# yusuke1127/RoboManipBaselines

Measured on AMD Instinct MI355X. Metric: env-steps/s (whole node) + policy-inference us/step, MujocoUR5eCable x N ACT, higher is better.
Workload: dtype f64 physics + fp32 policy

## Files before the change

### include/rmbx.h

```cpp
#ifndef RMBX_H_
#define RMBX_H_

#include <stddef.h>
#include <stdint.h>

#ifdef __cplusplus
extern "C" {
#endif

#define RMBX_OK 0
#define RMBX_ERR_ARG -1
#define RMBX_ERR_HIP -2
#define RMBX_ERR_STATE -3

#define RMBX_ABI_VERSION 2

int rmbx_abi_version(void);
const char* rmbx_last_error(void);
int rmbx_device_count(int* count);

int rmbx_act_ensemble(const float* new_chunk, const uint8_t* push, const uint8_t* active,
                      float* hist, int32_t* hist_len, int32_t* hist_head,
                      const double* w_table, const double* dn_scale, const double* dn_sub,
                      const double* dn_add, double* out, int n_env, int chunk, int adim,
// ... 368 lines not shown
int rmbx_split_bf16x3(const float* x, void* planes, long long n, void* stream);
int rmbx_split_f16x2(const float* w, int N, int K, void* planes, float* scale, void* stream);
int rmbx_linear_f16x3(const float* a, long long lda, const void* w_planes, long long ldw, long long w_plane_stride,
                      const float* w_scale, const float* bias, float* c, long long ldc, int M, int N, int K, int relu,
                      void* stream);
int rmbx_linear_f16x3_batched(const float* a, long long lda, long long a_bs, const void* w_planes, long long ldw,
                              long long w_plane_stride, long long w_bs, const float* w_scale, long long ws_bs,
                              const float* bias, float* c, long long ldc, long long c_bs, int batch, int M, int N,
                              int K, int relu, void* stream);
int rmbx_linear_f16x3_presplit(const void* a_planes, long long lda, long long a_plane_stride, const float* a_rinv,
                               const void* w_planes, long long ldw, long long w_plane_stride, const float* w_scale,
                               const float* bias, const float* res, float* c, long long ldc, int M, int N, int K,
                               int relu, void* stream);
int rmbx_linear_f16x3_presplit_split(const void* a_planes, long long lda, long long a_plane_stride, const float* a_rinv,
                                     const float* a_norm, const void* w_planes, long long ldw, long long w_plane_stride,
                                     const float* w_scale, float w_norm_max, float b_abs_max, const float* bias,
                                     int relu, void* out_planes, long long ldo, long long out_plane_stride,
                                     float* out_rinv, int M, int N, int K, void* stream);
int rmbx_linear_f16x3_presplit_batched(const void* a_planes, long long lda, long long a_plane_stride, long long a_bs,
                                       const float* a_rinv, long long r_bs, const void* w_planes, long long ldw,
                                       long long w_plane_stride, long long w_bs, const float* w_scale, long long ws_bs,
                                       const float* bias, float* c, long long ldc, long long c_bs, int batch, int M,
                                       int N, int K, int relu, void* stream);
int rmbx_conv3x3_f16x3_patch(const float* in, int N, int H, int W, int C, const void* w_planes,
                             long long w_plane_stride, const float* w_scale, const float* bias, const float* res,
                             float* out, int Cout, int relu, void* stream);
int rmbx_conv2d_f16x3(const float* in, int N, int H, int W, int C, const void* w_planes, const float* w_scale,
                      const float* bias, const float* res, float* out, int Cout, int KH, int KW, int stride, int pad,
                      int relu, void* stream);
int rmbx_attention_f32x6(const float* q, const float* k, const float* v, float* out, int B, int heads, int Lq, int Lk,
                         long long q_bstride, int q_rstride, long long k_bstride, int k_rstride, long long v_bstride,
                         int v_rstride, float scale, void* stream);
int rmbx_attention_f16x3(const float* q, const float* k, const float* v, float* out, int* redo, int B, int heads,
                         int Lq, int Lk, long long q_bstride, int q_rstride, long long k_bstride, int k_rstride,
                         long long v_bstride, int v_rstride, float scale, void* stream);
int rmbx_groupnorm_act(const float* x, const float* weight, const float* bias, float* out, int B, int C, int T,
                       int groups, float eps, int mish, void* stream);
int rmbx_add_layernorm(const void* x, const void* r, const float* weight, const float* bias, void* out,
                       int rows, int D, float eps, int dtype, void* stream);
int rmbx_add_layernorm_pos(const void* x, const void* r, const float* weight, const float* bias, void* out,
                           const void* pos, int pos_rows, void* out_pos, int rows, int D, float eps, int dtype,
                           void* stream);
int rmbx_add_layernorm_split(const float* x, const float* r, const float* weight, const float* bias, float* out,
                             void* y_planes, float* y_rinv, float* y_norm, const float* pos, int pos_rows,
                             float* out_pos, void* pos_planes, float* pos_rinv, int rows, int D, float eps,
                             void* stream);
// ... 68 lines not shown
```

### robomanipbaselines_amd/_native.py

```python

import ctypes
import os

import numpy as np

_LIB_PATH = os.path.join(os.path.dirname(os.path.abspath(__file__)), "_lib",
                         f"librmbx_{os.environ['RMBX_LIB_VARIANT']}.so" if os.environ.get("RMBX_LIB_VARIANT")
                         else "librmbx.so")

_c_int = ctypes.c_int
_c_p = ctypes.c_void_p
_c_sz = ctypes.c_size_t
_c_d = ctypes.c_double

SIGNATURES = {
    "rmbx_abi_version": (_c_int, []),
    "rmbx_last_error": (ctypes.c_char_p, []),
    "rmbx_device_count": (_c_int, [_c_p]),
    "rmbx_act_ensemble": (
        _c_int,
        [_c_p] * 11 + [_c_int, _c_int, _c_int, _c_int, _c_p],
    ),
    "rmbx_cable_reward": (_c_int, [_c_p] * 5 + [_c_int, _c_int, _c_p]),
    "rmbx_door_reward": (_c_int, [_c_p, _c_p, _c_p, _c_p, _c_int, _c_d, _c_d, _c_p]),
# ... 59 lines not shown
    "rmbx_conv2d_direct_f32": (_c_int, [_c_p] + [_c_int] * 4 + [_c_p] * 3 + [_c_int] * 5 + [_c_p]),
    "rmbx_split_bf16x3": (_c_int, [_c_p, _c_p, ctypes.c_longlong, _c_p]),
    "rmbx_split_f16x2": (_c_int, [_c_p, _c_int, _c_int, _c_p, _c_p, _c_p]),
    "rmbx_linear_f16x3": (_c_int, [_c_p, ctypes.c_longlong, _c_p, ctypes.c_longlong, ctypes.c_longlong, _c_p, _c_p,
                                   _c_p, ctypes.c_longlong, _c_int, _c_int, _c_int, _c_int, _c_p]),
    "rmbx_linear_f16x3_batched": (_c_int, [_c_p, ctypes.c_longlong, ctypes.c_longlong, _c_p, ctypes.c_longlong,
                                           ctypes.c_longlong, ctypes.c_longlong, _c_p, ctypes.c_longlong, _c_p, _c_p,
                                           ctypes.c_longlong, ctypes.c_longlong] + [_c_int] * 5 + [_c_p]),
    "rmbx_conv3x3_f16x3_patch": (_c_int, [_c_p] + [_c_int] * 4 + [_c_p, ctypes.c_longlong] + [_c_p] * 4
                                 + [_c_int, _c_int, _c_p]),
    "rmbx_conv2d_f16x3": (_c_int, [_c_p] + [_c_int] * 4 + [_c_p] * 5 + [_c_int] * 6 + [_c_p]),
    "rmbx_add_layernorm": (_c_int, [_c_p] * 5 + [_c_int, _c_int, ctypes.c_float, _c_int, _c_p]),
    "rmbx_groupnorm_act": (_c_int, [_c_p] * 4 + [_c_int] * 4 + [ctypes.c_float, _c_int, _c_p]),
    "rmbx_add_layernorm_split": (_c_int, [_c_p] * 9 + [_c_int, _c_p, _c_p, _c_p, _c_int, _c_int, ctypes.c_float, _c_p]),
    "rmbx_linear_f16x3_presplit_split": (_c_int, [_c_p, ctypes.c_longlong, ctypes.c_longlong, _c_p, _c_p, _c_p,
                                                  ctypes.c_longlong, ctypes.c_longlong, _c_p, ctypes.c_float,
                                                  ctypes.c_float, _c_p, _c_int, _c_p, ctypes.c_longlong,
                                                  ctypes.c_longlong, _c_p, _c_int, _c_int, _c_int, _c_p]),
    "rmbx_linear_f16x3_presplit_batched": (_c_int, [_c_p, ctypes.c_longlong, ctypes.c_longlong, ctypes.c_longlong, _c_p,
                                                    ctypes.c_longlong, _c_p, ctypes.c_longlong, ctypes.c_longlong,
                                                    ctypes.c_longlong, _c_p, ctypes.c_longlong, _c_p, _c_p,
                                                    ctypes.c_longlong, ctypes.c_longlong, _c_int, _c_int, _c_int, _c_int,
                                                    _c_int, _c_p]),
    "rmbx_wino4_input_split": (_c_int, [_c_p, _c_int, _c_int, _c_int, _c_int, _c_p, _c_p, _c_p]),
    "rmbx_linear_f16x3_presplit": (_c_int, [_c_p, ctypes.c_longlong, ctypes.c_longlong, _c_p, _c_p, ctypes.c_longlong,
                                            ctypes.c_longlong, _c_p, _c_p, _c_p, _c_p, ctypes.c_longlong, _c_int, _c_int,
                                            _c_int, _c_int, _c_p]),
    "rmbx_add_layernorm_pos": (_c_int, [_c_p] * 6 + [_c_int, _c_p, _c_int, _c_int, ctypes.c_float, _c_int, _c_p]),
    "rmbx_ddpm_step": (_c_int, [_c_p] * 4 + [_c_sz, _c_p, _c_p]),
    "rmbx_ddim_step": (_c_int, [_c_p] * 3 + [_c_sz, _c_p, _c_int, _c_p]),
    "rmbx_philox_normal": (_c_int, [ctypes.c_uint64, _c_p, _c_p, _c_int, _c_int, _c_p, _c_int, _c_int, _c_int, _c_p]),
    "rmbx_image_perturb": (_c_int, [_c_p, _c_p, _c_p, _c_int, _c_p, ctypes.c_uint64, _c_p, _c_p, _c_int, _c_p, _c_int,
                                    _c_int, _c_int, _c_p]),
    "rmbx_action_perturb": (_c_int, [_c_p] * 7 + [ctypes.c_uint64, _c_p, _c_p, _c_p, _c_int, _c_int, _c_p]),
    "rmbx_resize_crop_u8": (_c_int, [_c_p] + [_c_int] * 10 + [ctypes.c_float, ctypes.c_float, _c_p, _c_int, _c_p]),
    "rmbx_resize_f32": (_c_int, [_c_p, _c_p] + [_c_int] * 5 + [_c_p]),
    "rmbx_pointcloud_fps": (_c_int, [_c_p, _c_p, _c_int, _c_int, _c_int, _c_d, _c_p, _c_p, _c_int, _c_int,
                                     _c_p, _c_p, _c_p, _c_p, _c_p, _c_p, _c_p]),
    "rmbx_sarnn_attention": (_c_int, [_c_p] * 8 + [_c_int] * 4 + [ctypes.c_float, _c_p]),
    "rmbx_sarnn_lstm_step": (_c_int, [_c_p] * 12 + [_c_int] * 4 + [_c_p]),
}


class Camera(ctypes.Structure):

    _fields_ = [("body", ctypes.c_int32), ("width", ctypes.c_int32), ("height", ctypes.c_int32),
# ... 204 lines not shown
```

### robomanipbaselines_amd/csrc/rmbx_gemm.hip

```cpp
#include "rmbx_common.h"

#include <cstdint>
#include <cstdlib>
#include <type_traits>

namespace rmbx {
namespace {

typedef short bf16x8 __attribute__((ext_vector_type(8)));
typedef _Float16 f16x8 __attribute__((ext_vector_type(8)));
typedef float f32x4v __attribute__((ext_vector_type(4)));
typedef __bf16 bf16x2v __attribute__((ext_vector_type(2)));
typedef _Float16 f16x2v __attribute__((ext_vector_type(2)));
typedef float f32x2v __attribute__((ext_vector_type(2)));

constexpr int GM_BM = 256, GM_BN = 128, GM_BK = 32;
constexpr int GM_THREADS = 512;
constexpr int GM_A_PLANE = GM_BM * GM_BK * 2;
constexpr int GM_GROUP = 8;
template <int BN>
constexpr int gm_b_plane() { return BN * GM_BK * 2; }
template <int PC, int BN = 128>
constexpr int gm_stage() { return PC * (GM_A_PLANE + gm_b_plane<BN>()); }
template <int BN>
// ... 1 lines not shown
template <int PC, int BN = 128, int NS = 2>
constexpr int gm_smem() {
  return (NS * gm_stage<PC, BN>() > gm_epi_bytes<BN>() ? NS * gm_stage<PC, BN>() : gm_epi_bytes<BN>()) +
         (PC == 2 ? 1024 + 64 : 0);
}
static_assert(gm_smem<3>() <= 160 * 1024 && gm_smem<2, 128, 3>() <= 160 * 1024 && gm_smem<2, 64, 3>() <= 160 * 1024 &&
                  gm_smem<2, 256, 2>() <= 160 * 1024,
              "the LDS of a CU");

struct GemmArgs {
  const float* A;
  const uint16_t* W;
  const float* bias;
  float* C;
  long long lda, ldc, ldw, wps;
  int M, N, K, relu;
  int tiles_m, tiles_n;
  const float* res;
  int ih, iw, ic, oh, ow, kw, stride, pad;
  int batch;
  long long a_bs, w_bs, c_bs;
  const float* ws;
  long long ws_bs;
};

__device__ __forceinline__ uint32_t pk_bf16(float x, float y) {
  f32x2v v = {x, y};
  return __builtin_bit_cast(uint32_t, __builtin_convertvector(v, bf16x2v));
}

__device__ __forceinline__ void split_pair(float x, float y, uint32_t& p0, uint32_t& p1, uint32_t& p2) {
  p0 = pk_bf16(x, y);
  const float rx = x - __uint_as_float(p0 << 16), ry = y - __uint_as_float(p0 & 0xffff0000u);
  p1 = pk_bf16(rx, ry);
  const float sx = rx - __uint_as_float(p1 << 16), sy = ry - __uint_as_float(p1 & 0xffff0000u);
  p2 = pk_bf16(sx, sy);
}

__device__ __forceinline__ uint32_t pk_f16(float x, float y) {
  f32x2v v = {x, y};
  return __builtin_bit_cast(uint32_t, __builtin_convertvector(v, f16x2v));
}

__device__ __forceinline__ void split_f16_pair(float x, float y, uint32_t& h, uint32_t& l) {
  h = pk_f16(x, y);
  const f16x2v hv = __builtin_bit_cast(f16x2v, h);
  l = pk_f16((x - (float)hv[0]) * 2048.f, (y - (float)hv[1]) * 2048.f);
// ... 33 lines not shown
  R[1] = __builtin_bit_cast(float4, v1);
  R[2] = __builtin_bit_cast(float4, v2);
  R[3] = __builtin_bit_cast(float4, v3);
}

template <bool CONV, int VAR = 0, int PC = 3, int BN = 128>
__global__ void __launch_bounds__(GM_THREADS, 1) gemm_f32x6_kernel(GemmArgs g) {
  static_assert(PC == 3 || PC == 2, "bf16x6 (3 pieces) or f16x3 (2 pieces)");
  static_assert(BN == 128 || ((BN == 64 || BN == 256) && PC == 2), "BN = 64 / 256: the f16x3 form's tiles");
  static_assert(BN != 256 || (VAR & 1024) == 0, "the 256-wide tile runs two stages");
  constexpr int GROUP = ((VAR >> 1) & 3) == 1 ? 4 : ((VAR >> 1) & 3) == 2 ? 16 : GM_GROUP;
  constexpr int STAGE = gm_stage<PC, BN>(), A_BYTES = PC * GM_A_PLANE, B_PLANE = gm_b_plane<BN>();
  constexpr int NJ = BN / 32;
  constexpr int WP = PC * BN / 128;
  constexpr int PPP = BN / 16;
  constexpr int W_OPS = WP, A_OPS = 4, A_ROWS = 2;
  static_assert(A_OPS == 2 * A_ROWS, "two 16-byte loads (8 f32 of one k quarter) per staged row");
  constexpr int NS = (PC == 2 && (VAR & 1024) != 0) ? 3 : 2;
  constexpr int SMEM = gm_smem<PC, BN, NS>();
  __shared__ __attribute__((aligned(16))) unsigned char smem[SMEM];
  const int tid = threadIdx.x, lane = tid & 63, wave = tid >> 6;
  const int wm = wave & 3, wn = wave >> 2;

  const int nblk = gridDim.x, bid = blockIdx.x;
  const int xcd = bid & 7, q = nblk >> 3, r = nblk & 7;
  int lin = (xcd < r ? xcd * (q + 1) : r * (q + 1) + (xcd - r) * q) + (bid >> 3);
  if (g.batch > 1) {
    const int per_item = g.tiles_m * g.tiles_n;
    const int item = lin / per_item;
    lin -= item * per_item;
    g.A += item * g.a_bs;
    g.W += item * g.w_bs;
    g.C += item * g.c_bs;
    if (g.ws) g.ws += item * g.ws_bs;
  }
  const int per_group = GROUP * g.tiles_n;
  const int first_m = (lin / per_group) * GROUP;
  const int gsize = min(g.tiles_m - first_m, GROUP);
  const int in_group = lin - (lin / per_group) * per_group;
  const int tm = first_m + in_group % gsize, tn = in_group / gsize;
  const int m0 = tm * GM_BM, n0 = tn * BN;

  const int aq = tid & 3, arow = tid >> 2;
  const float* ag0 = g.A + (long long)min(m0 + arow, g.M - 1) * g.lda + 8 * aq;
  const float* ag1 = g.A + (long long)min(m0 + arow + 128, g.M - 1) * g.lda + 8 * aq;
  const int aoff0 = arow * 64 + ((aq ^ ((arow >> 2) & 2)) << 4);
  const int aoff1 = (arow + 128) * 64 + ((aq ^ (((arow + 128) >> 2) & 2)) << 4);
  const uint16_t* bsrc[WP];
#pragma unroll
  for (int t = 0; t < WP; ++t) {
    const int i = wave * WP + t, p = i / PPP;
    const int row = (i % PPP) * 16 + (lane >> 2);
    const int sl = (lane & 3) ^ ((row >> 2) & 2);
    bsrc[t] = g.W + p * g.wps + (long long)(n0 + row) * g.ldw + sl * 8;
  }
  auto stage_b = [&](int kt, int buf) {
    if constexpr ((VAR & 512) != 0) {
      if (kt > 0) return;
    }
    unsigned char* base = smem + buf * STAGE + A_BYTES;
#pragma unroll
    for (int t = 0; t < W_OPS; ++t) glds16(bsrc[t] + kt * GM_BK, base + (wave * WP + t) * 1024);
  };
  long long cbase[2] = {0, 0};
  int cy[2] = {0, 0}, cx[2] = {0, 0};
  if constexpr (CONV) {
#pragma unroll
    for (int r2 = 0; r2 < 2; ++r2) {
      const int m = min(m0 + arow + 128 * r2, g.M - 1);
      const int hw = g.oh * g.ow;
      const int img = m / hw, rem = m - img * hw;
      const int oy = rem / g.ow, ox = rem - oy * g.ow;
      cy[r2] = oy * g.stride - g.pad;
      cx[r2] = ox * g.stride - g.pad;
      cbase[r2] = ((long long)(img * g.ih + cy[r2]) * g.iw + cx[r2]) * g.ic + 8 * aq;
    }
  }
// ... 129 lines not shown
          c = __builtin_amdgcn_mfma_f32_16x16x32_bf16(a[i][0], b[nj][0], c, 0, 0, 0);
          acc[2 * h + i][nj] = c;
        }
      }
  };
  auto read_b = [&](bf16x8 (&b)[NJ][PC], int buf) {
    const unsigned char* Bs = smem + buf * STAGE + A_BYTES;
#pragma unroll
    for (int nj = 0; nj < NJ; ++nj) {
      const int off = frag_off(wn * (BN / 2) + nj * 16 + fr);
#pragma unroll
      for (int p = 0; p < PC; ++p) b[nj][p] = *(const bf16x8*)(Bs + p * B_PLANE + off);
    }
  };

  const int KT = g.K / GM_BK;
  constexpr bool SKIPS = (VAR & (256 | 512)) != 0;
  constexpr int LEAD = NS - 1;
  constexpr int SPLIT_WAIT = SKIPS ? 0 : W_OPS + A_OPS;
  constexpr int END_WAIT = SKIPS ? 0 : (NS == 3 ? W_OPS + A_OPS : A_OPS);
  static_assert(SPLIT_WAIT <= 63 && END_WAIT <= 63, "vmcnt holds 6 bits on gfx950");
  static_assert(SKIPS || (END_WAIT < SPLIT_WAIT || NS == 3), "a stage's DMA is retired after the A split");
  auto stage_of = [](int k) { return NS == 2 ? (k & 1) : k % 3; };
  auto k_loop = [&](auto scaled) {
    float4 Ra[4], Rb[4];
    int oka, okb;
    if constexpr (NS == 3) {
      stage_b(0, 0);
      oka = load_a(Ra, 0);
      stage_b(min(1, KT - 1), 1);
      okb = load_a(Rb, min(1, KT - 1));
    } else {
      oka = load_a(Ra, 0);
      stage_b(0, 0);
      okb = load_a(Rb, min(1, KT - 1));
    }
    wait_vm_regs<SPLIT_WAIT>(Ra);
    store_a(Ra, oka, 0, scaled);
    wait_vm<END_WAIT>();
    asm volatile("s_waitcnt lgkmcnt(0)\n\ts_barrier" ::: "memory");
    auto step = [&](int kt, float4 (&Rcur)[4], int& okcur, float4 (&Rnext)[4], int& oknext) {
      const int buf = stage_of(kt), nbuf = stage_of(kt + 1);
      const bool more = kt + 1 < KT;
      stage_b(min(kt + LEAD, KT - 1), stage_of(kt + LEAD));
      oknext = load_a(Rnext, min(kt + 2, KT - 1));
      if constexpr (BN == 256) {
        const unsigned char* S = smem + buf * STAGE;
        f16x8 ah[4], al[4];
#pragma unroll
        for (int mi = 0; mi < 4; ++mi) {
          const int off = frag_off(wm * 64 + mi * 16 + fr);
          ah[mi] = __builtin_bit_cast(f16x8, *(const bf16x8*)(S + off));
          al[mi] = __builtin_bit_cast(f16x8, *(const bf16x8*)(S + GM_A_PLANE + off));
        }
        auto wide_half = [&](int hh) {
#pragma unroll
          for (int q = 0; q < NJ / 2; ++q) {
            const int nj = hh * (NJ / 2) + q;
            const int off = frag_off(wn * (BN / 2) + nj * 16 + fr);
            const f16x8 bh = __builtin_bit_cast(f16x8, *(const bf16x8*)(S + A_BYTES + off));
            const f16x8 bl = __builtin_bit_cast(f16x8, *(const bf16x8*)(S + A_BYTES + B_PLANE + off));
            const f16x8 bsc = bh * (_Float16)0.00048828125f;
#pragma unroll
            for (int mi = 0; mi < 4; ++mi) {
              f32x4v c = acc[mi][nj];
              c = __builtin_amdgcn_mfma_f32_16x16x32_f16(al[mi], bsc, c, 0, 0, 0);
              c = __builtin_amdgcn_mfma_f32_16x16x32_f16(ah[mi], bl, c, 0, 0, 0);
              c = __builtin_amdgcn_mfma_f32_16x16x32_f16(ah[mi], bh, c, 0, 0, 0);
              acc[mi][nj] = c;
            }
          }
        };
        wide_half(0);
        wait_vm_regs<SPLIT_WAIT>(Rcur);
        store_a(Rcur, okcur, nbuf, scaled);
        wide_half(1);
        wait_vm<END_WAIT>();
        if (more) asm volatile("s_waitcnt lgkmcnt(0)\n\ts_barrier" ::: "memory");
// ... 11 lines not shown
        wait_vm_regs<SPLIT_WAIT>(Rcur);
        store_a(Rcur, okcur, nbuf, scaled);
      }
      if constexpr (VAR & 1) __builtin_amdgcn_s_setprio(1);
      half_step(buf, 0, b, bs);
      if constexpr (VAR & 1) __builtin_amdgcn_s_setprio(0);
      if (late) {
        wait_vm_regs<SPLIT_WAIT>(Rcur);
        store_a(Rcur, okcur, nbuf, scaled);
      }
      if constexpr (VAR & 1) __builtin_amdgcn_s_setprio(1);
      half_step(buf, 1, b, bs);
      if constexpr (VAR & 1) __builtin_amdgcn_s_setprio(0);
      wait_vm<END_WAIT>();
      if (more) asm volatile("s_waitcnt lgkmcnt(0)\n\ts_barrier" ::: "memory");
    };
    for (int kt = 0; kt < KT; kt += 2) {
      step(kt, Rb, okb, Ra, oka);
      if (kt + 1 < KT) step(kt + 1, Ra, oka, Rb, okb);
    }
    wait_vm_regs<0>(Ra);
    wait_vm_regs<0>(Rb);
  };
  k_loop(std::false_type{});

  if constexpr (PC == 2) {
    uint32_t b0 = amax0, b1 = amax1;
    b0 = max(b0, (uint32_t)__shfl_xor((int)b0, 1));
    b0 = max(b0, (uint32_t)__shfl_xor((int)b0, 2));
    b1 = max(b1, (uint32_t)__shfl_xor((int)b1, 1));
    b1 = max(b1, (uint32_t)__shfl_xor((int)b1, 2));
    const float m0 = __uint_as_float(b0), m1 = __uint_as_float(b1);
    float inv0 = 1.f, inv1 = 1.f;
    auto row_scale = [](float m, float& sc, float& inv) {
      if ((m > 32768.f || (m > 0.f && m < 0.015625f)) && m <= 3.4e38f) {
        int e;
        frexpf(m, &e);
        sc = ldexpf(1.f, 14 - e);
        inv = ldexpf(1.f, e - 14);
        return true;
      }
      return false;
    };
    const bool need = row_scale(m0, as0, inv0) | row_scale(m1, as1, inv1);
    float* rinv = reinterpret_cast<float*>(smem + SMEM - 1024 - 64);
    int* flag = reinterpret_cast<int*>(smem + SMEM - 64);
    if (aq == 0) {
      rinv[arow] = inv0;
      rinv[arow + 128] = inv1;
    }
    const unsigned long long bal = __ballot(need);
    if (lane == 0) flag[wave] = bal != 0ull;
    asm volatile("s_waitcnt vmcnt(0) lgkmcnt(0)\n\ts_barrier" ::: "memory");
    int any = 0;
#pragma unroll
    for (int w = 0; w < 8; ++w) any |= flag[w];
    if (any) {
      zero_acc();
      k_loop(std::true_type{});
    }
    if (any) {
#pragma unroll
      for (int i = 0; i < 4; ++i)
#pragma unroll
        for (int e = 0; e < 4; ++e) {
          const float inv = rinv[wm * 64 + i * 16 + 4 * fs + e];
#pragma unroll
          for (int j = 0; j < NJ; ++j) acc[i][j][e] *= inv;
        }
    }
  }

  if constexpr ((VAR & 16) != 0) {
    asm volatile("s_waitcnt lgkmcnt(0)\n\ts_barrier" ::: "memory");
    constexpr int WC = BN / 2 < 64 ? BN / 2 : 64, PITCH = WC + 4;
    constexpr int LPR = WC / 4, RPI = 64 / LPR;
    constexpr int NPASS = (BN / 2) / WC, NJP = NJ / NPASS;
    float* T = reinterpret_cast<float*>(smem) + wave * (64 * PITCH);
#pragma unroll
    for (int pass = 0; pass < NPASS; ++pass) {
    if (pass > 0) asm volatile("s_waitcnt lgkmcnt(0)" ::: "memory");
#pragma unroll
    for (int mi = 0; mi < 4; ++mi)
#pragma unroll
      for (int q = 0; q < NJP; ++q)
#pragma unroll
        for (int e = 0; e < 4; ++e) T[(mi * 16 + 4 * fs + e) * PITCH + q * 16 + fr] = acc[mi][pass * NJP + q][e];
    asm volatile("s_waitcnt lgkmcnt(0)" ::: "memory");
    const int c4 = (lane % LPR) * 4;
    const int n = n0 + wn * (BN / 2) + pass * WC + c4;
    float4 bn = make_float4(0.f, 0.f, 0.f, 0.f);
    if (g.bias) bn = *(const float4*)(g.bias + n);
    float4 sn = make_float4(1.f, 1.f, 1.f, 1.f);
    if constexpr (PC == 2) sn = *(const float4*)(g.ws + n);
#pragma unroll
    for (int it = 0; it < 64 / RPI; ++it) {
      const int r = it * RPI + lane / LPR;
      const int m = m0 + wm * 64 + r;
      if (m < g.M) {
        float4 v = *(const float4*)(T + r * PITCH + c4);
        if constexpr (PC == 2) {
          v.x *= sn.x; v.y *= sn.y; v.z *= sn.z; v.w *= sn.w;
        }
        v.x += bn.x; v.y += bn.y; v.z += bn.z; v.w += bn.w;
        if (g.res) {
          const float4 rv = *(const float4*)(g.res + (long long)m * g.ldc + n);
          v.x += rv.x; v.y += rv.y; v.z += rv.z; v.w += rv.w;
        }
        if (g.relu) {
          v.x = fmaxf(v.x, 0.f); v.y = fmaxf(v.y, 0.f); v.z = fmaxf(v.z, 0.f); v.w = fmaxf(v.w, 0.f);
        }
        *(float4*)(g.C + (long long)m * g.ldc + n) = v;
      }
    }
    }
    return;
  }
#pragma unroll
  for (int nj = 0; nj < NJ; ++nj) {
    const int n = n0 + wn * (BN / 2) + nj * 16 + fr;
    const float bn = g.bias ? g.bias[n] : 0.f;
    const float sn = PC == 2 ? g.ws[n] : 1.f;
#pragma unroll
    for (int mi = 0; mi < 4; ++mi) {
      const int mb = m0 + wm * 64 + mi * 16 + 4 * fs;
#pragma unroll
      for (int e = 0; e < 4; ++e) {
        const int m = mb + e;
        if (!(VAR & 8) && m < g.M) {
          float v = acc[mi][nj][e];
          if constexpr (PC == 2) v *= sn;
          v += bn;
          if (g.res) v += g.res[(long long)m * g.ldc + n];
          if (g.relu) v = fmaxf(v, 0.f);
          g.C[(long long)m * g.ldc + n] = v;
        }
      }
    }
  }
}
// ... 497 lines not shown
  uint16_t* planes;
  long long ldo, ps;
  float* rinv;
  const float* a_norm;
  float w_norm_max, b_abs_max;
};

template <int GROUP, int VAR = 0, bool SPLIT_OUT = false>
__global__ void __launch_bounds__(GM_THREADS, 1) gemm_f16x3_presplit3_kernel(GemmArgs g, const uint16_t* __restrict__ Ap,
                                                                            long long aps, long long ldah,
                                                                            const float* __restrict__ arinv,
                                                                            PresplitOut po = PresplitOut{},
                                                                            long long a_bs = 0, long long r_bs = 0) {
  constexpr int BN = 256, NJ = 8;
  constexpr int A_STAGE = 2 * GM_A_PLANE, B_PLANE = gm_b_plane<BN>(), W_STAGE = 2 * B_PLANE;
  constexpr int W_RING = 3 * A_STAGE;
  constexpr int SMEM = 3 * A_STAGE + 2 * W_STAGE;
  static_assert(SMEM == 160 * 1024 && gm_epi_bytes<BN>() <= SMEM, "the LDS of a CU");
  constexpr int APW = 2 * (GM_BM / 16) / 8, WPW = 2 * (BN / 16) / 8;
  static_assert(APW == 4 && WPW == 4 && APW + WPW == NJ, "one DMA issue per column-tile MFMA group");
  __shared__ __attribute__((aligned(16))) unsigned char smem[SMEM];
  const int tid = threadIdx.x, lane = tid & 63, wave = tid >> 6;
  const int wm = wave & 3, wn = wave >> 2;
  const int nblk = gridDim.x, bid = blockIdx.x;
  const int xcd = bid & 7, q = nblk >> 3, r = nblk & 7;
  int lin = (xcd < r ? xcd * (q + 1) : r * (q + 1) + (xcd - r) * q) + (bid >> 3);
  if (g.batch > 1) {
    const int per_item = g.tiles_m * g.tiles_n;
    const int item = lin / per_item;
    lin -= item * per_item;
    Ap += item * a_bs;
    arinv += item * r_bs;
    g.W += item * g.w_bs;
    g.C += item * g.c_bs;
    g.ws += item * g.ws_bs;
  }
  const int per_group = GROUP * g.tiles_n;
  const int first_m = (lin / per_group) * GROUP;
  const int gsize = min(g.tiles_m - first_m, GROUP);
  const int in_group = lin - (lin / per_group) * per_group;
  const int tm = first_m + in_group % gsize, tn = in_group / gsize;
  const int m0 = tm * GM_BM, n0 = tn * BN;
  const bool dead = n0 + wn * (BN / 2) >= g.N;

  const uint16_t* asrc[APW];
  const uint16_t* wsrc[WPW];
  int adst[APW], wdst[WPW];
#pragma unroll
  for (int t = 0; t < APW; ++t) {
    const int i = wave * APW + t, p = i / 16, rb = i % 16, row = rb * 16 + (lane >> 2);
    const int sl = (lane & 3) ^ ((row >> 2) & 2);
    asrc[t] = Ap + p * aps + (long long)min(m0 + row, g.M - 1) * ldah + sl * 8;
    adst[t] = p * GM_A_PLANE + rb * 1024;
  }
#pragma unroll
  for (int t = 0; t < WPW; ++t) {
    const int i = wave * WPW + t, p = i / 16, rb = i % 16, row = rb * 16 + (lane >> 2);
    const int sl = (lane & 3) ^ ((row >> 2) & 2);
    wsrc[t] = g.W + p * g.wps + (long long)min(n0 + row, g.N - 1) * g.ldw + sl * 8;
    wdst[t] = W_RING + p * B_PLANE + rb * 1024;
  }
  auto dma_a = [&](int t, int kt) {
    if constexpr ((VAR & 1) == 0) glds16(asrc[t] + kt * GM_BK, smem + (kt % 3) * A_STAGE + adst[t]);
  };
  auto dma_w = [&](int t, int kt) {
    if constexpr ((VAR & 1) == 0) glds16(wsrc[t] + kt * GM_BK, smem + (kt & 1) * W_STAGE + wdst[t]);
  };

  f32x4v acc[4][NJ];
#pragma unroll
  for (int i = 0; i < 4; ++i)
#pragma unroll
    for (int j = 0; j < NJ; ++j) acc[i][j] = (f32x4v){0.f, 0.f, 0.f, 0.f};
  const int fr = lane & 15, fs = lane >> 4;
  auto frag_off = [&](int row) { return row * 64 + ((fs ^ ((row >> 2) & 2)) << 4); };

  const int KT = g.K / GM_BK;
#pragma unroll
  for (int t = 0; t < WPW; ++t) glds16(wsrc[t], smem + wdst[t]);
#pragma unroll
  for (int t = 0; t < APW; ++t) glds16(asrc[t], smem + adst[t]);
  if (KT > 1) {
// ... 203 lines not shown
}

extern "C" int rmbx_split_bf16x3(const float* x, void* planes, long long n, void* stream) {
  RMBX_CHECK_ARG(x && planes && n >= 0, "rmbx_split_bf16x3: bad arguments");
  if (n == 0) return RMBX_OK;
  const long long blocks = (n + 255) / 256;
  hipLaunchKernelGGL(rmbx::split_bf16x3_kernel, dim3((unsigned)(blocks < 65536 ? blocks : 65536)), dim3(256), 0,
                     (hipStream_t)stream, x, (uint16_t*)planes, n);
  RMBX_CHECK_LAUNCH();
  return RMBX_OK;
}

namespace rmbx {
namespace {
static int gemm_cus() {
  static const int cus = [] {
    int dev = 0, n = 0;
    if (hipGetDevice(&dev) != hipSuccess || hipDeviceGetAttribute(&n, hipDeviceAttributeMultiprocessorCount, dev) != hipSuccess)
      return 256;
    return n > 0 ? n : 256;
  }();
  return cus;
}
template <bool CONV>
void launch_f16x3(const GemmArgs& g, hipStream_t st, int bn) {
  const char* we = getenv("RMBX_GEMM_WIDE");
  const bool wide = !(we && atoi(we) == 0);
  const int n256 = g.N / 256 * 256;
  const long long items = g.batch > 1 ? g.batch : 1;
  const char* fe = getenv("RMBX_GEMM_FILL");
  if (!(fe && atoi(fe) == 0) && bn == GM_BN) {
    const long long cus = gemm_cus();
    const long long wide_blocks = (long long)g.tiles_m * (g.N / 256 + (g.N % 256 ? 1 : 0)) * items;
    if (wide_blocks < cus) {
      int nb = GM_BN;
      if ((long long)g.tiles_m * (g.N / GM_BN) * items < cus && g.N % 64 == 0) nb = 64;
      GemmArgs t = g;
      t.tiles_n = g.N / nb;
      launch_gemm<CONV, 2>((long long)t.tiles_m * t.tiles_n * items, t, st, nb);
      return;
    }
  }
  if (!wide || bn != GM_BN || n256 == 0) {
    launch_gemm<CONV, 2>((long long)g.tiles_m * g.tiles_n * items, g, st, bn);
    return;
  }
  GemmArgs w = g;
  w.N = n256;
  w.tiles_n = n256 / 256;
  launch_gemm<CONV, 2>((long long)w.tiles_m * w.tiles_n * items, w, st, 256);
  if (n256 == g.N) return;
  GemmArgs t = g;
  t.W = g.W + (long long)n256 * g.ldw;
  t.bias = g.bias ? g.bias + n256 : nullptr;
  t.C = g.C + n256;
  t.res = g.res ? g.res + n256 : nullptr;
  t.ws = g.ws + n256;
  t.N = g.N - n256;
  t.tiles_n = t.N / GM_BN;
  launch_gemm<CONV, 2>((long long)t.tiles_m * t.tiles_n * items, t, st, GM_BN);
}

template <int PC>
int linear_impl(const char* fn, const float* a, long long lda, long long a_bs, const void* w_planes, long long ldw,
                long long wps, long long w_bs, const float* ws, long long ws_bs, const float* bias, float* c,
                long long ldc, long long c_bs, int batch, int M, int N, int K, int relu, void* stream) {
  RMBX_CHECK_ARG(a && w_planes && c && (PC == 3 || ws), "%s: null pointer", fn);
  RMBX_CHECK_ARG(batch >= 1 && M >= 0 && N > 0 && K > 0, "%s: bad shape M=%d N=%d K=%d", fn, M, N, K);
  const int bn = PC == 2 && N % GM_BN != 0 ? 64 : GM_BN;
  RMBX_CHECK_ARG(N % bn == 0, "%s: N=%d must be a multiple of %d", fn, N, PC == 2 ? 64 : GM_BN);
  RMBX_CHECK_ARG(K % GM_BK == 0, "%s: K=%d must be a multiple of %d", fn, K, GM_BK);
  RMBX_CHECK_ARG(lda >= K && lda % 4 == 0 && a_bs % 4 == 0 && ldc >= N && ldw >= K && ldw % 8 == 0 && wps % 8 == 0 &&
                     w_bs % 8 == 0,
// ... 118 lines not shown
                 "%s: bad strides lda=%lld ldw=%lld ldc=%lld", fn, lda, ldw, ldc);
  RMBX_CHECK_ARG(((uintptr_t)a_planes | (uintptr_t)w_planes | (uintptr_t)c | (uintptr_t)bias | (uintptr_t)res |
                  (uintptr_t)w_scale) % 16 == 0,
                 "%s: operands must be 16-B aligned", fn);
  RMBX_CHECK_ARG((long long)M * lda + a_plane_stride < (1ll << 62), "%s: too large", fn);
  if (M == 0) return RMBX_OK;
  rmbx::GemmArgs g{nullptr, (const uint16_t*)w_planes, bias, c, 0, ldc, ldw, w_plane_stride, M, N, K, relu ? 1 : 0,
                   (M + rmbx::GM_BM - 1) / rmbx::GM_BM, 0, res};
  g.batch = 1;
  g.ws = w_scale;
  hipStream_t st = (hipStream_t)stream;
  const uint16_t* ap = (const uint16_t*)a_planes;
  g.tiles_n = (N + 255) / 256;
  const long long blocks = (long long)g.tiles_m * g.tiles_n;
  RMBX_CHECK_ARG(blocks < (1ll << 31), "%s: too many tiles", fn);
  const char* ge = getenv("RMBX_PRESPLIT_GROUP");
  const int grp = ge ? atoi(ge) : 8;
  const char* ve = getenv("RMBX_PRESPLIT_VAR");
  const int var = ve ? atoi(ve) : 0;
  const char* fe = getenv("RMBX_PRESPLIT_FORM");
  const int form = fe ? atoi(fe) : 3;
  const bool form2 = form == 2;
  if (!form2) {
    switch (var) {
      case 0: hipLaunchKernelGGL((rmbx::gemm_f16x3_presplit3_kernel<8, 0>), dim3((unsigned)blocks), dim3(rmbx::GM_THREADS), 0, st, g, ap, a_plane_stride, lda, a_rinv); break;
      case 1: hipLaunchKernelGGL((rmbx::gemm_f16x3_presplit3_kernel<8, 1>), dim3((unsigned)blocks), dim3(rmbx::GM_THREADS), 0, st, g, ap, a_plane_stride, lda, a_rinv); break;
      case 2: hipLaunchKernelGGL((rmbx::gemm_f16x3_presplit3_kernel<8, 2>), dim3((unsigned)blocks), dim3(rmbx::GM_THREADS), 0, st, g, ap, a_plane_stride, lda, a_rinv); break;
      case 4: hipLaunchKernelGGL((rmbx::gemm_f16x3_presplit3_kernel<8, 4>), dim3((unsigned)blocks), dim3(rmbx::GM_THREADS), 0, st, g, ap, a_plane_stride, lda, a_rinv); break;
      case 5: hipLaunchKernelGGL((rmbx::gemm_f16x3_presplit3_kernel<8, 5>), dim3((unsigned)blocks), dim3(rmbx::GM_THREADS), 0, st, g, ap, a_plane_stride, lda, a_rinv); break;
      case 6: hipLaunchKernelGGL((rmbx::gemm_f16x3_presplit3_kernel<8, 6>), dim3((unsigned)blocks), dim3(rmbx::GM_THREADS), 0, st, g, ap, a_plane_stride, lda, a_rinv); break;
      case 8: hipLaunchKernelGGL((rmbx::gemm_f16x3_presplit3_kernel<8, 8>), dim3((unsigned)blocks), dim3(rmbx::GM_THREADS), 0, st, g, ap, a_plane_stride, lda, a_rinv); break;
      default: RMBX_CHECK_ARG(false, "%s: RMBX_PRESPLIT_VAR %d", fn, var);
    }
    RMBX_CHECK_LAUNCH();
    return RMBX_OK;
  }
  if (var != 0) {
    switch (var) {
      case 1: hipLaunchKernelGGL((rmbx::gemm_f16x3_presplit_kernel<256, 8, 1>), dim3((unsigned)blocks), dim3(rmbx::GM_THREADS), 0, st, g, ap, a_plane_stride, lda, a_rinv); break;
      case 2: hipLaunchKernelGGL((rmbx::gemm_f16x3_presplit_kernel<256, 8, 2>), dim3((unsigned)blocks), dim3(rmbx::GM_THREADS), 0, st, g, ap, a_plane_stride, lda, a_rinv); break;
      case 4: hipLaunchKernelGGL((rmbx::gemm_f16x3_presplit_kernel<256, 8, 4>), dim3((unsigned)blocks), dim3(rmbx::GM_THREADS), 0, st, g, ap, a_plane_stride, lda, a_rinv); break;
      case 5: hipLaunchKernelGGL((rmbx::gemm_f16x3_presplit_kernel<256, 8, 5>), dim3((unsigned)blocks), dim3(rmbx::GM_THREADS), 0, st, g, ap, a_plane_stride, lda, a_rinv); break;
      case 6: hipLaunchKernelGGL((rmbx::gemm_f16x3_presplit_kernel<256, 8, 6>), dim3((unsigned)blocks), dim3(rmbx::GM_THREADS), 0, st, g, ap, a_plane_stride, lda, a_rinv); break;
      default: RMBX_CHECK_ARG(false, "%s: RMBX_PRESPLIT_VAR %d", fn, var);
    }
    RMBX_CHECK_LAUNCH();
    return RMBX_OK;
  }
  switch (grp) {
    case 2: hipLaunchKernelGGL((rmbx::gemm_f16x3_presplit_kernel<256, 2>), dim3((unsigned)blocks), dim3(rmbx::GM_THREADS), 0, st, g, ap, a_plane_stride, lda, a_rinv); break;
    case 4: hipLaunchKernelGGL((rmbx::gemm_f16x3_presplit_kernel<256, 4>), dim3((unsigned)blocks), dim3(rmbx::GM_THREADS), 0, st, g, ap, a_plane_stride, lda, a_rinv); break;
    case 16: hipLaunchKernelGGL((rmbx::gemm_f16x3_presplit_kernel<256, 16>), dim3((unsigned)blocks), dim3(rmbx::GM_THREADS), 0, st, g, ap, a_plane_stride, lda, a_rinv); break;
    default: hipLaunchKernelGGL((rmbx::gemm_f16x3_presplit_kernel<256, 8>), dim3((unsigned)blocks), dim3(rmbx::GM_THREADS), 0, st, g, ap, a_plane_stride, lda, a_rinv);
  }
// ... 7 lines not shown
                                                float w_norm_max, float b_abs_max, const float* bias, int relu,
                                                void* out_planes, long long ldo, long long out_plane_stride,
                                                float* out_rinv, int M, int N, int K, void* stream) {
  const char* fn = "rmbx_linear_f16x3_presplit_split";
  RMBX_CHECK_ARG(a_planes && a_rinv && a_norm && w_planes && w_scale && out_planes && out_rinv, "%s: null pointer", fn);
  RMBX_CHECK_ARG(M >= 0 && N > 0 && K > 0 && N % rmbx::GM_BN == 0 && K % rmbx::GM_BK == 0,
                 "%s: bad shape M=%d N=%d K=%d (N %% 128, K %% 32)", fn, M, N, K);
  RMBX_CHECK_ARG(lda >= K && lda % 8 == 0 && a_plane_stride % 8 == 0 && ldw >= K && ldw % 8 == 0 &&
                     w_plane_stride % 8 == 0 && ldo >= N && ldo % 8 == 0 && out_plane_stride % 8 == 0 &&
                     out_plane_stride >= (long long)M * ldo,
                 "%s: bad strides lda=%lld ldw=%lld ldo=%lld", fn, lda, ldw, ldo);
  RMBX_CHECK_ARG(((uintptr_t)a_planes | (uintptr_t)w_planes | (uintptr_t)bias | (uintptr_t)w_scale |
                  (uintptr_t)out_planes) % 16 == 0,
                 "%s: operands must be 16-B aligned", fn);
  RMBX_CHECK_ARG(w_norm_max >= 0.f && b_abs_max >= 0.f, "%s: bad bounds", fn);
  if (M == 0) return RMBX_OK;
  rmbx::GemmArgs g{nullptr, (const uint16_t*)w_planes, bias, nullptr, 0, 0, ldw, w_plane_stride, M, N, K,
                   relu ? 1 : 0, (M + rmbx::GM_BM - 1) / rmbx::GM_BM, (N + 255) / 256, nullptr};
  g.batch = 1;
  g.ws = w_scale;
  const long long blocks = (long long)g.tiles_m * g.tiles_n;
  RMBX_CHECK_ARG(blocks < (1ll << 31), "%s: too many tiles", fn);
  rmbx::PresplitOut po{(uint16_t*)out_planes, ldo, out_plane_stride, out_rinv, a_norm, w_norm_max, b_abs_max};
  hipLaunchKernelGGL((rmbx::gemm_f16x3_presplit3_kernel<8, 0, true>), dim3((unsigned)blocks), dim3(rmbx::GM_THREADS), 0,
                     (hipStream_t)stream, g, (const uint16_t*)a_planes, a_plane_stride, lda, a_rinv, po);
  RMBX_CHECK_LAUNCH();
  return RMBX_OK;
}

extern "C" int rmbx_linear_f16x3_presplit_batched(const void* a_planes, long long lda, long long a_plane_stride,
                                                  long long a_bs, const float* a_rinv, long long r_bs,
                                                  const void* w_planes, long long ldw, long long w_plane_stride,
                                                  long long w_bs, const float* w_scale, long long ws_bs,
                                                  const float* bias, float* c, long long ldc, long long c_bs,
                                                  int batch, int M, int N, int K, int relu, void* stream) {
  const char* fn = "rmbx_linear_f16x3_presplit_batched";
  RMBX_CHECK_ARG(a_planes && a_rinv && w_planes && w_scale && c && batch >= 1, "%s: null pointer / batch", fn);
  RMBX_CHECK_ARG(M >= 0 && N > 0 && K > 0 && N % rmbx::GM_BN == 0 && K % rmbx::GM_BK == 0,
                 "%s: bad shape M=%d N=%d K=%d (N %% 128, K %% 32)", fn, M, N, K);
  RMBX_CHECK_ARG(lda >= K && lda % 8 == 0 && a_plane_stride % 8 == 0 && a_bs % 8 == 0 && ldw >= K && ldw % 8 == 0 &&
                     w_plane_stride % 8 == 0 && w_bs % 8 == 0 && ws_bs % 4 == 0 && ldc >= N && ldc % 4 == 0 &&
                     c_bs % 4 == 0 && r_bs >= 0,
                 "%s: bad strides", fn);
  RMBX_CHECK_ARG(((uintptr_t)a_planes | (uintptr_t)w_planes | (uintptr_t)c | (uintptr_t)bias | (uintptr_t)w_scale) % 16 ==
                     0,
                 "%s: operands must be 16-B aligned", fn);
  if (M == 0) return RMBX_OK;
  rmbx::GemmArgs g{nullptr, (const uint16_t*)w_planes, bias, c, 0, ldc, ldw, w_plane_stride, M, N, K, relu ? 1 : 0,
                   (M + rmbx::GM_BM - 1) / rmbx::GM_BM, (N + 255) / 256, nullptr};
  g.batch = batch;
  g.w_bs = w_bs;
  g.c_bs = c_bs;
  g.ws = w_scale;
  g.ws_bs = ws_bs;
  const long long blocks = (long long)g.tiles_m * g.tiles_n * batch;
  RMBX_CHECK_ARG(blocks < (1ll << 31), "%s: too many tiles", fn);
  hipLaunchKernelGGL((rmbx::gemm_f16x3_presplit3_kernel<8, 0, false>), dim3((unsigned)blocks), dim3(rmbx::GM_THREADS), 0,
                     (hipStream_t)stream, g, (const uint16_t*)a_planes, a_plane_stride, lda, a_rinv, rmbx::PresplitOut{},
                     a_bs, r_bs);
  RMBX_CHECK_LAUNCH();
  return RMBX_OK;
}
```

Baseline: 22860.

## Split tail-wave GEMM tiles into half-width blocks to balance the last wave

When the tile count leaves a partial last wave (remainder at most half the CU count), the last R wide 256-column tiles are each split into two 128-column half-blocks, launching R extra blocks. The aim is to shorten the tail wave on the wide and presplit f16x3 GEMM kernels. Waves whose half falls outside the column limit skip the MFMA and fragment loads through a compile-time dead path and exit before the epilogue. This adds per-block index remapping and duplicated A-tile loads for the split tiles, and it can be turned off with an environment variable.

Result: no change. 22820 (-0.2%).

```diff
diff --git a/include/rmbx.h b/include/rmbx.h
--- a/include/rmbx.h
+++ b/include/rmbx.h
@@ -414,6 +414,7 @@
                                        long long w_plane_stride, long long w_bs, const float* w_scale, long long ws_bs,
                                        const float* bias, float* c, long long ldc, long long c_bs, int batch, int M,
                                        int N, int K, int relu, void* stream);
+int rmbx_gemm_tail_plan(long long tiles, int* tail);
 int rmbx_conv3x3_f16x3_patch(const float* in, int N, int H, int W, int C, const void* w_planes,
                              long long w_plane_stride, const float* w_scale, const float* bias, const float* res,
                              float* out, int Cout, int relu, void* stream);
diff --git a/robomanipbaselines_amd/_native.py b/robomanipbaselines_amd/_native.py
--- a/robomanipbaselines_amd/_native.py
+++ b/robomanipbaselines_amd/_native.py
@@ -105,6 +105,7 @@
                                                     ctypes.c_longlong, _c_p, ctypes.c_longlong, _c_p, _c_p,
                                                     ctypes.c_longlong, ctypes.c_longlong, _c_int, _c_int, _c_int, _c_int,
                                                     _c_int, _c_p]),
+    "rmbx_gemm_tail_plan": (_c_int, [ctypes.c_longlong, _c_p]),
     "rmbx_wino4_input_split": (_c_int, [_c_p, _c_int, _c_int, _c_int, _c_int, _c_p, _c_p, _c_p]),
     "rmbx_linear_f16x3_presplit": (_c_int, [_c_p, ctypes.c_longlong, ctypes.c_longlong, _c_p, _c_p, ctypes.c_longlong,
                                             ctypes.c_longlong, _c_p, _c_p, _c_p, _c_p, ctypes.c_longlong, _c_int, _c_int,
diff --git a/robomanipbaselines_amd/csrc/rmbx_gemm.hip b/robomanipbaselines_amd/csrc/rmbx_gemm.hip
--- a/robomanipbaselines_amd/csrc/rmbx_gemm.hip
+++ b/robomanipbaselines_amd/csrc/rmbx_gemm.hip
@@ -47,7 +47,24 @@
   long long a_bs, w_bs, c_bs;
   const float* ws;
   long long ws_bs;
+  int tail;
 };
+
+struct TileBlock {
+  int bid, nblk;
+  int half;
+};
+__device__ __forceinline__ TileBlock tile_block(int tail) {
+  TileBlock b{(int)blockIdx.x, (int)gridDim.x - tail, -1};
+  const int first = b.nblk - tail;
+  if (b.bid >= first) {
+    const int j = b.bid - first, u = j >> 4, v = j & 15;
+    const int w = min(tail - 8 * u, 8);
+    b.half = v >= w ? 1 : 0;
+    b.bid = first + 8 * u + v - b.half * w;
+  }
+  return b;
+}
 
 __device__ __forceinline__ uint32_t pk_bf16(float x, float y) {
   f32x2v v = {x, y};
@@ -127,7 +144,11 @@
   const int tid = threadIdx.x, lane = tid & 63, wave = tid >> 6;
   const int wm = wave & 3, wn = wave >> 2;
 
-  const int nblk = gridDim.x, bid = blockIdx.x;
+  int nblk = gridDim.x, bid = blockIdx.x, half = -1;
+  if constexpr (BN == 256) {
+    const TileBlock tb = tile_block(g.tail);
+    nblk = tb.nblk, bid = tb.bid, half = tb.half;
+  }
   const int xcd = bid & 7, q = nblk >> 3, r = nblk & 7;
   int lin = (xcd < r ? xcd * (q + 1) : r * (q + 1) + (xcd - r) * q) + (bid >> 3);
   if (g.batch > 1) {
@@ -144,7 +165,9 @@
   const int gsize = min(g.tiles_m - first_m, GROUP);
   const int in_group = lin - (lin / per_group) * per_group;
   const int tm = first_m + in_group % gsize, tn = in_group / gsize;
-  const int m0 = tm * GM_BM, n0 = tn * BN;
+  const int m0 = tm * GM_BM, n0 = tn * BN + (half > 0 ? BN / 2 : 0);
+  const int nlim = BN == 256 && half >= 0 ? n0 + BN / 2 : g.N;
+  const bool dead = BN == 256 && __builtin_amdgcn_readfirstlane(n0 + wn * (BN / 2) >= nlim);
 
   const int aq = tid & 3, arow = tid >> 2;
   const float* ag0 = g.A + (long long)min(m0 + arow, g.M - 1) * g.lda + 8 * aq;
@@ -157,7 +180,8 @@
     const int i = wave * WP + t, p = i / PPP;
     const int row = (i % PPP) * 16 + (lane >> 2);
     const int sl = (lane & 3) ^ ((row >> 2) & 2);
-    bsrc[t] = g.W + p * g.wps + (long long)(n0 + row) * g.ldw + sl * 8;
+    const int wrow = BN == 256 ? min(n0 + row, nlim - 1) : n0 + row;
+    bsrc[t] = g.W + p * g.wps + (long long)wrow * g.ldw + sl * 8;
   }
   auto stage_b = [&](int kt, int buf) {
     if constexpr ((VAR & 512) != 0) {
@@ -333,7 +357,7 @@
   static_assert(SPLIT_WAIT <= 63 && END_WAIT <= 63, "vmcnt holds 6 bits on gfx950");
   static_assert(SKIPS || (END_WAIT < SPLIT_WAIT || NS == 3), "a stage's DMA is retired after the A split");
   auto stage_of = [](int k) { return NS == 2 ? (k & 1) : k % 3; };
-  auto k_loop = [&](auto scaled) {
+  auto k_loop = [&](auto scaled, auto dead_c) {
     float4 Ra[4], Rb[4];
     int oka, okb;
     if constexpr (NS == 3) {
@@ -358,13 +382,16 @@
       if constexpr (BN == 256) {
         const unsigned char* S = smem + buf * STAGE;
         f16x8 ah[4], al[4];
-#pragma unroll
-        for (int mi = 0; mi < 4; ++mi) {
-          const int off = frag_off(wm * 64 + mi * 16 + fr);
-          ah[mi] = __builtin_bit_cast(f16x8, *(const bf16x8*)(S + off));
-          al[mi] = __builtin_bit_cast(f16x8, *(const bf16x8*)(S + GM_A_PLANE + off));
+        if constexpr (!decltype(dead_c)::value) {
+#pragma unroll
+          for (int mi = 0; mi < 4; ++mi) {
+            const int off = frag_off(wm * 64 + mi * 16 + fr);
+            ah[mi] = __builtin_bit_cast(f16x8, *(const bf16x8*)(S + off));
+            al[mi] = __builtin_bit_cast(f16x8, *(const bf16x8*)(S + GM_A_PLANE + off));
+          }
         }
         auto wide_half = [&](int hh) {
+          if constexpr (decltype(dead_c)::value) return;
 #pragma unroll
           for (int q = 0; q < NJ / 2; ++q) {
             const int nj = hh * (NJ / 2) + q;
@@ -422,7 +449,16 @@
     wait_vm_regs<0>(Ra);
     wait_vm_regs<0>(Rb);
   };
-  k_loop(std::false_type{});
+  auto run_k = [&](auto scaled) {
+    if constexpr (BN == 256) {
+      if (dead) {
+        k_loop(scaled, std::true_type{});
+        return;
+      }
+    }
+    k_loop(scaled, std::false_type{});
+  };
+  run_k(std::false_type{});
 
   if constexpr (PC == 2) {
     uint32_t b0 = amax0, b1 = amax1;
@@ -457,7 +493,7 @@
     for (int w = 0; w < 8; ++w) any |= flag[w];
     if (any) {
       zero_acc();
-      k_loop(std::true_type{});
+      run_k(std::true_type{});
     }
     if (any) {
 #pragma unroll
@@ -473,6 +509,7 @@
 
   if constexpr ((VAR & 16) != 0) {
     asm volatile("s_waitcnt lgkmcnt(0)\n\ts_barrier" ::: "memory");
+    if (dead) return;
     constexpr int WC = BN / 2 < 64 ? BN / 2 : 64, PITCH = WC + 4;
     constexpr int LPR = WC / 4, RPI = 64 / LPR;
     constexpr int NPASS = (BN / 2) / WC, NJP = NJ / NPASS;
@@ -516,6 +553,7 @@
     }
     return;
   }
+  if (dead) return;
 #pragma unroll
   for (int nj = 0; nj < NJ; ++nj) {
     const int n = n0 + wn * (BN / 2) + nj * 16 + fr;
@@ -1059,7 +1097,8 @@
   __shared__ __attribute__((aligned(16))) unsigned char smem[SMEM];
   const int tid = threadIdx.x, lane = tid & 63, wave = tid >> 6;
   const int wm = wave & 3, wn = wave >> 2;
-  const int nblk = gridDim.x, bid = blockIdx.x;
+  const TileBlock tb = tile_block(g.tail);
+  const int nblk = tb.nblk, bid = tb.bid;
   const int xcd = bid & 7, q = nblk >> 3, r = nblk & 7;
   int lin = (xcd < r ? xcd * (q + 1) : r * (q + 1) + (xcd - r) * q) + (bid >> 3);
   if (g.batch > 1) {
@@ -1077,8 +1116,9 @@
   const int gsize = min(g.tiles_m - first_m, GROUP);
   const int in_group = lin - (lin / per_group) * per_group;
   const int tm = first_m + in_group % gsize, tn = in_group / gsize;
-  const int m0 = tm * GM_BM, n0 = tn * BN;
-  const bool dead = n0 + wn * (BN / 2) >= g.N;
+  const int m0 = tm * GM_BM, n0 = tn * BN + (tb.half > 0 ? BN / 2 : 0);
+  const int nlim = tb.half >= 0 ? min(n0 + BN / 2, g.N) : g.N;
+  const bool dead = n0 + wn * (BN / 2) >= nlim;
 
   const uint16_t* asrc[APW];
   const uint16_t* wsrc[WPW];
@@ -1094,7 +1134,7 @@
   for (int t = 0; t < WPW; ++t) {
     const int i = wave * WPW + t, p = i / 16, rb = i % 16, row = rb * 16 + (lane >> 2);
     const int sl = (lane & 3) ^ ((row >> 2) & 2);
-    wsrc[t] = g.W + p * g.wps + (long long)min(n0 + row, g.N - 1) * g.ldw + sl * 8;
+    wsrc[t] = g.W + p * g.wps + (long long)min(n0 + row, nlim - 1) * g.ldw + sl * 8;
     wdst[t] = W_RING + p * B_PLANE + rb * 1024;
   }
   auto dma_a = [&](int t, int kt) {
@@ -1344,6 +1384,17 @@
   }();
   return cus;
 }
+static int gemm_slots() {
+  const char* se = getenv("RMBX_GEMM_TAIL_SLOTS");
+  const int n = se ? atoi(se) : 0;
+  return n > 0 ? n : gemm_cus();
+}
+static int gemm_tail(long long tiles) {
+  const char* te = getenv("RMBX_GEMM_TAIL");
+  if (te && atoi(te) == 0) return 0;
+  const long long slots = gemm_slots(), R = tiles % slots;
+  return R > 0 && 2 * R <= slots ? (int)R : 0;
+}
 template <bool CONV>
 void launch_f16x3(const GemmArgs& g, hipStream_t st, int bn) {
   const char* we = getenv("RMBX_GEMM_WIDE");
@@ -1352,7 +1403,7 @@
   const long long items = g.batch > 1 ? g.batch : 1;
   const char* fe = getenv("RMBX_GEMM_FILL");
   if (!(fe && atoi(fe) == 0) && bn == GM_BN) {
-    const long long cus = gemm_cus();
+    const long long cus = gemm_slots();
     const long long wide_blocks = (long long)g.tiles_m * (g.N / 256 + (g.N % 256 ? 1 : 0)) * items;
     if (wide_blocks < cus) {
       int nb = GM_BN;
@@ -1370,7 +1421,9 @@
   GemmArgs w = g;
   w.N = n256;
   w.tiles_n = n256 / 256;
-  launch_gemm<CONV, 2>((long long)w.tiles_m * w.tiles_n * items, w, st, 256);
+  const long long wtiles = (long long)w.tiles_m * w.tiles_n * items;
+  w.tail = gemm_tail(wtiles);
+  launch_gemm<CONV, 2>(wtiles + w.tail, w, st, 256);
   if (n256 == g.N) return;
   GemmArgs t = g;
   t.W = g.W + (long long)n256 * g.ldw;
@@ -1535,14 +1588,15 @@
   const int form = fe ? atoi(fe) : 3;
   const bool form2 = form == 2;
   if (!form2) {
+    g.tail = rmbx::gemm_tail(blocks);
     switch (var) {
-      case 0: hipLaunchKernelGGL((rmbx::gemm_f16x3_presplit3_kernel<8, 0>), dim3((unsigned)blocks), dim3(rmbx::GM_THREADS), 0, st, g, ap, a_plane_stride, lda, a_rinv); break;
-      case 1: hipLaunchKernelGGL((rmbx::gemm_f16x3_presplit3_kernel<8, 1>), dim3((unsigned)blocks), dim3(rmbx::GM_THREADS), 0, st, g, ap, a_plane_stride, lda, a_rinv); break;
-      case 2: hipLaunchKernelGGL((rmbx::gemm_f16x3_presplit3_kernel<8, 2>), dim3((unsigned)blocks), dim3(rmbx::GM_THREADS), 0, st, g, ap, a_plane_stride, lda, a_rinv); break;
-      case 4: hipLaunchKernelGGL((rmbx::gemm_f16x3_presplit3_kernel<8, 4>), dim3((unsigned)blocks), dim3(rmbx::GM_THREADS), 0, st, g, ap, a_plane_stride, lda, a_rinv); break;
-      case 5: hipLaunchKernelGGL((rmbx::gemm_f16x3_presplit3_kernel<8, 5>), dim3((unsigned)blocks), dim3(rmbx::GM_THREADS), 0, st, g, ap, a_plane_stride, lda, a_rinv); break;
-      case 6: hipLaunchKernelGGL((rmbx::gemm_f16x3_presplit3_kernel<8, 6>), dim3((unsigned)blocks), dim3(rmbx::GM_THREADS), 0, st, g, ap, a_plane_stride, lda, a_rinv); break;
-      case 8: hipLaunchKernelGGL((rmbx::gemm_f16x3_presplit3_kernel<8, 8>), dim3((unsigned)blocks), dim3(rmbx::GM_THREADS), 0, st, g, ap, a_plane_stride, lda, a_rinv); break;
+      case 0: hipLaunchKernelGGL((rmbx::gemm_f16x3_presplit3_kernel<8, 0>), dim3((unsigned)(blocks + g.tail)), dim3(rmbx::GM_THREADS), 0, st, g, ap, a_plane_stride, lda, a_rinv); break;
+      case 1: hipLaunchKernelGGL((rmbx::gemm_f16x3_presplit3_kernel<8, 1>), dim3((unsigned)(blocks + g.tail)), dim3(rmbx::GM_THREADS), 0, st, g, ap, a_plane_stride, lda, a_rinv); break;
+      case 2: hipLaunchKernelGGL((rmbx::gemm_f16x3_presplit3_kernel<8, 2>), dim3((unsigned)(blocks + g.tail)), dim3(rmbx::GM_THREADS), 0, st, g, ap, a_plane_stride, lda, a_rinv); break;
+      case 4: hipLaunchKernelGGL((rmbx::gemm_f16x3_presplit3_kernel<8, 4>), dim3((unsigned)(blocks + g.tail)), dim3(rmbx::GM_THREADS), 0, st, g, ap, a_plane_stride, lda, a_rinv); break;
+      case 5: hipLaunchKernelGGL((rmbx::gemm_f16x3_presplit3_kernel<8, 5>), dim3((unsigned)(blocks + g.tail)), dim3(rmbx::GM_THREADS), 0, st, g, ap, a_plane_stride, lda, a_rinv); break;
+      case 6: hipLaunchKernelGGL((rmbx::gemm_f16x3_presplit3_kernel<8, 6>), dim3((unsigned)(blocks + g.tail)), dim3(rmbx::GM_THREADS), 0, st, g, ap, a_plane_stride, lda, a_rinv); break;
+      case 8: hipLaunchKernelGGL((rmbx::gemm_f16x3_presplit3_kernel<8, 8>), dim3((unsigned)(blocks + g.tail)), dim3(rmbx::GM_THREADS), 0, st, g, ap, a_plane_stride, lda, a_rinv); break;
       default: RMBX_CHECK_ARG(false, "%s: RMBX_PRESPLIT_VAR %d", fn, var);
     }
     RMBX_CHECK_LAUNCH();
@@ -1596,7 +1650,8 @@
   const long long blocks = (long long)g.tiles_m * g.tiles_n;
   RMBX_CHECK_ARG(blocks < (1ll << 31), "%s: too many tiles", fn);
   rmbx::PresplitOut po{(uint16_t*)out_planes, ldo, out_plane_stride, out_rinv, a_norm, w_norm_max, b_abs_max};
-  hipLaunchKernelGGL((rmbx::gemm_f16x3_presplit3_kernel<8, 0, true>), dim3((unsigned)blocks), dim3(rmbx::GM_THREADS), 0,
+  g.tail = rmbx::gemm_tail(blocks);
+  hipLaunchKernelGGL((rmbx::gemm_f16x3_presplit3_kernel<8, 0, true>), dim3((unsigned)(blocks + g.tail)), dim3(rmbx::GM_THREADS), 0,
                      (hipStream_t)stream, g, (const uint16_t*)a_planes, a_plane_stride, lda, a_rinv, po);
   RMBX_CHECK_LAUNCH();
   return RMBX_OK;
@@ -1629,9 +1684,16 @@
   g.ws_bs = ws_bs;
   const long long blocks = (long long)g.tiles_m * g.tiles_n * batch;
   RMBX_CHECK_ARG(blocks < (1ll << 31), "%s: too many tiles", fn);
-  hipLaunchKernelGGL((rmbx::gemm_f16x3_presplit3_kernel<8, 0, false>), dim3((unsigned)blocks), dim3(rmbx::GM_THREADS), 0,
+  g.tail = rmbx::gemm_tail(blocks);
+  hipLaunchKernelGGL((rmbx::gemm_f16x3_presplit3_kernel<8, 0, false>), dim3((unsigned)(blocks + g.tail)), dim3(rmbx::GM_THREADS), 0,
                      (hipStream_t)stream, g, (const uint16_t*)a_planes, a_plane_stride, lda, a_rinv, rmbx::PresplitOut{},
                      a_bs, r_bs);
   RMBX_CHECK_LAUNCH();
   return RMBX_OK;
 }
+
+extern "C" int rmbx_gemm_tail_plan(long long tiles, int* tail) {
+  RMBX_CHECK_ARG(tail && tiles >= 0 && tiles < (1ll << 31), "rmbx_gemm_tail_plan: bad arguments");
+  *tail = rmbx::gemm_tail(tiles);
+  return RMBX_OK;
+}
```
